# tzt101/MichiGAN

Hardware: NVIDIA H100
Metric: 512x512 images/sec (generator forward) (higher is better)
Workload: dtype fp16/bf16 tensor-core operands (bf16 hi+lo split where needed), fp32 accumulate and storage

## Files before the change

### michigan_b200/csrc/mg_aux.cu

```cuda
#include <cuda_runtime.h>
#include <cstdint>
#include <cmath>
#include <cstdlib>
#include <cuda_fp16.h>
#include <cuda_bf16.h>
#include "mg_internal.h"

namespace mg {

__device__ __forceinline__ float rtf32(float x) {
    uint32_t r;
    asm("cvt.rna.tf32.f32 %0, %1;\n" : "=r"(r) : "f"(x));
    return __uint_as_float(r);
}
__device__ __forceinline__ float act_fn(float v, int act) {
    if (act == MG_ACT_RELU) return fmaxf(v, 0.f);
    if (act == MG_ACT_LRELU) return v > 0.f ? v : 0.2f * v;
    if (act == MG_ACT_TANH) return tanhf(v);
    return v;
}
__device__ __forceinline__ void split16(float v, int fmt, uint16_t& hi, uint16_t& lo) {
    if (fmt == 1) {
        const __half h = __float2half_rn(fminf(fmaxf(v, -65504.f), 65504.f));
        hi = __half_as_ushort(h);
        lo = __half_as_ushort(__float2half_rn(v - __half2float(h)));
    } else {
        const __nv_bfloat16 h = __float2bfloat16_rn(v);
        hi = __bfloat16_as_ushort(h);
        lo = __bfloat16_as_ushort(__float2bfloat16_rn(v - __bfloat162float(h)));
    }
}
static inline int cdiv(long long a, long long b) { return (int)((a + b - 1) / b); }

__global__ void pack_weight_kernel(const float* __restrict__ w, float* __restrict__ out, int O, int I, int KH, int KW,
                                   const float* __restrict__ inv_sigma, int round_) {
    const long long total = (long long)O * KH * KW * I;
    const float s = inv_sigma ? *inv_sigma : 1.f;
    for (long long idx = blockIdx.x * (long long)blockDim.x + threadIdx.x; idx < total;
         idx += (long long)gridDim.x * blockDim.x) {
        const int i = idx % I;
        long long t = idx / I;
        const int kw = t % KW; t /= KW;
        const int kh = t % KH;
        const int o = t / KH;
        float v = w[(((long long)o * I + i) * KH + kh) * KW + kw] * s;
        out[idx] = round_ ? rtf32(v) : v;
    }
}

__global__ void pack_weight_gb_kernel(const float* __restrict__ wg, const float* __restrict__ wb,
                                      float* __restrict__ out, int C, int I, int KH, int KW, int BN) {
    const long long total = 2LL * C * KH * KW * I;
    const int half = BN / 2;
    for (long long idx = blockIdx.x * (long long)blockDim.x + threadIdx.x; idx < total;
         idx += (long long)gridDim.x * blockDim.x) {
        const int i = idx % I;
        long long t = idx / I;
        const int kw = t % KW; t /= KW;
        const int kh = t % KH;
        const int R = t / KH;
        const int tile = R / BN, rr = R % BN;
        const float* src = rr < half ? wg : wb;
        const int c = tile * half + (rr < half ? rr : rr - half);
        out[idx] = rtf32(src[(((long long)c * I + i) * KH + kh) * KW + kw]);
    }
}

__global__ void pack_weight16_kernel(const float* __restrict__ w, uint16_t* __restrict__ out, int O, int I, int KH, int KW,
                                     const float* __restrict__ inv_sigma, int fmt, int split) {
    const long long total = (long long)O * KH * KW * I;
    const float s = inv_sigma ? *inv_sigma : 1.f;
    const int parts = split ? 2 : 1;
    for (long long idx = blockIdx.x * (long long)blockDim.x + threadIdx.x; idx < total;
         idx += (long long)gridDim.x * blockDim.x) {
        const int i = idx % I;
        long long t = idx / I;
        const int kw = t % KW; t /= KW;
        const int kh = t % KH;
        const int o = t / KH;
        const float v = w[(((long long)o * I + i) * KH + kh) * KW + kw] * s;
        uint16_t hi, lo;
        split16(v, fmt, hi, lo);
        const size_t base = ((size_t)o * KH * KW + (size_t)(kh * KW + kw)) * parts * I;
        out[base + i] = hi;
        if (split) out[base + I + i] = lo;
    }
}
__global__ void pack_weight_gb16_kernel(const float* __restrict__ wg, const float* __restrict__ wb, uint16_t* __restrict__ out,
                                        int C, int I, int KH, int KW, int BN, int fmt, int split) {
    const long long total = 2LL * C * KH * KW * I;
    const int half = BN / 2;
    for (long long idx = blockIdx.x * (long long)blockDim.x + threadIdx.x; idx < total;
         idx += (long long)gridDim.x * blockDim.x) {
        const int i = idx % I;
        long long t = idx / I;
        const int kw = t % KW; t /= KW;
        const int kh = t % KH;
        const int R = t / KH;
        const int tile = R / BN, rr = R % BN;
        const float* src = rr < half ? wg : wb;
        const int c = tile * half + (rr < half ? rr : rr - half);
        uint16_t hi, lo;
        split16(src[(((long long)c * I + i) * KH + kh) * KW + kw], fmt, hi, lo);
        if (!split) {
            out[idx] = hi;
        } else {
            const size_t base = ((size_t)R * KH * KW + (size_t)(kh * KW + kw)) * 2 * I;
            out[base + i] = hi;
            out[base + I + i] = lo;
        }
    }
}

__global__ void pack_weight_thin_kernel(const float* __restrict__ w, float* __restrict__ out, int O, int I, int CinP,
                                        int KH, int KW) {
    const int total = KH * KW * CinP * O;
    for (int idx = blockIdx.x * blockDim.x + threadIdx.x; idx < total; idx += gridDim.x * blockDim.x) {
        const int o = idx % O;
        int t = idx / O;
        const int ci = t % CinP;
        const int tap = t / CinP;
        const int kh = tap / KW, kw = tap % KW;
        out[idx] = ci < I ? w[(((long long)o * I + ci) * KH + kh) * KW + kw] : 0.f;
    }
}

template <int CINP, int CPL>
__global__ void __launch_bounds__(256)
thin_conv_kernel(const mg_thin_args a, int tiles_w, int tiles_h, int num_tiles) {
    extern __shared__ __align__(16) float sm[];
    const int KH = a.KH, KW = a.KW, s = a.stride;
    const int Cout = a.Cout;
    const int PH = 7 * s + KH, PW = 15 * s + KW;
    float* w_s = sm;
    float* in_s = sm + KH * KW * CINP * Cout;
    const int nw = KH * KW * CINP * Cout;
    for (int i = threadIdx.x * 4; i < nw; i += blockDim.x * 4)
        *reinterpret_cast<float4*>(w_s + i) = __ldg(reinterpret_cast<const float4*>(a.w + i));

    const int warp = threadIdx.x >> 5, lane = threadIdx.x & 31;
    const int R = a.seg_resize > 0 ? a.seg_resize : 1;
    const int IH = a.H, IW = a.W;
    const int c_base = lane * CPL;
    const bool lane_active = c_base < Cout;

    for (int tile = blockIdx.x; tile < num_tiles; tile += gridDim.x) {
        const int tw = tile % tiles_w;
        const int th = (tile / tiles_w) % tiles_h;
        const int n = tile / (tiles_w * tiles_h);
        const int oh0 = th * 8, ow0 = tw * 16;
        const int ih0 = oh0 * s - a.pad, iw0 = ow0 * s - a.pad;
        __syncthreads();
        for (int i = threadIdx.x; i < PH * PW; i += blockDim.x) {
            const int py = i / PW, px = i - py * PW;
            int ih = ih0 + py, iw = iw0 + px;
            bool ok = true;
            if (a.pad_mode == 1) {
                if (ih < 0) ih = -ih;
                if (ih >= IH) ih = 2 * IH - 2 - ih;
                if (iw < 0) iw = -iw;
                if (iw >= IW) iw = 2 * IW - 2 - iw;
                ok = ih >= 0 && ih < IH && iw >= 0 && iw < IW;
            } else {
                ok = ih >= 0 && ih < IH && iw >= 0 && iw < IW;
            }
            float4 v0 = make_float4(0.f, 0.f, 0.f, 0.f), v1 = v0;
            if (ok) {
                const float* src = a.in + (((size_t)n * IH * R + (size_t)ih * R) * ((size_t)IW * R) + (size_t)iw * R) * CINP;
                v0 = __ldg(reinterpret_cast<const float4*>(src));
                if (CINP == 8) v1 = __ldg(reinterpret_cast<const float4*>(src + 4));
            }
            *reinterpret_cast<float4*>(in_s + (size_t)i * CINP) = v0;
            if (CINP == 8) *reinterpret_cast<float4*>(in_s + (size_t)i * CINP + 4) = v1;
        }
        __syncthreads();

        const int oh = oh0 + warp;
#pragma unroll 1
        for (int g = 0; g < 2; ++g) {
            float acc[8][CPL];
#pragma unroll
            for (int p_ = 0; p_ < 8; ++p_)
#pragma unroll
                for (int c = 0; c < CPL; ++c) acc[p_][c] = 0.f;
            if (lane_active) {
                for (int kh = 0; kh < KH; ++kh) {
                    const float* row = in_s + (size_t)((warp * s + kh) * PW) * CINP;
                    for (int kw = 0; kw < KW; ++kw) {
                        const float* wt = w_s + (size_t)((kh * KW + kw) * CINP) * Cout + c_base;
                        float wv[CINP][CPL];
#pragma unroll
                        for (int ci = 0; ci < CINP; ++ci) {
                            if constexpr (CPL == 4) {
                                const float4 t = *reinterpret_cast<const float4*>(wt + (size_t)ci * Cout);
                                wv[ci][0] = t.x; wv[ci][1] = t.y; wv[ci][2] = t.z; wv[ci][3] = t.w;
                            } else {
                                const float2 t = *reinterpret_cast<const float2*>(wt + (size_t)ci * Cout);
                                wv[ci][0] = t.x; wv[ci][1] = t.y;
                            }
                        }
#pragma unroll
                        for (int p_ = 0; p_ < 8; ++p_) {
                            const float* ip = row + (size_t)(((g * 8 + p_) * s + kw)) * CINP;
                            float iv[CINP];
                            const float4 t0 = *reinterpret_cast<const float4*>(ip);
                            iv[0] = t0.x; iv[1] = t0.y; iv[2] = t0.z; iv[3] = t0.w;
                            if constexpr (CINP == 8) {
                                const float4 t1 = *reinterpret_cast<const float4*>(ip + 4);
                                iv[4] = t1.x; iv[5] = t1.y; iv[6] = t1.z; iv[7] = t1.w;
                            }
#pragma unroll
                            for (int ci = 0; ci < CINP; ++ci)
#pragma unroll
                                for (int c = 0; c < CPL; ++c) acc[p_][c] = fmaf(iv[ci], wv[ci][c], acc[p_][c]);
                        }
                    }
                }
            }
            if (lane_active && oh < a.OH) {
                float bv[CPL];
#pragma unroll
                for (int c = 0; c < CPL; ++c) bv[c] = a.bias ? __ldg(a.bias + c_base + c) : 0.f;
#pragma unroll
                for (int p_ = 0; p_ < 8; ++p_) {
                    const int ow = ow0 + g * 8 + p_;
                    if (ow >= a.OW) continue;
                    const size_t pix = ((size_t)n * a.OH + oh) * a.OW + ow;
                    const float ps = a.pscale ? __ldg(a.pscale + pix) : 1.f;
                    const float pm = a.pmul ? __ldg(a.pmul + pix) : 1.f;
                    float y[CPL];
#pragma unroll
                    for (int c = 0; c < CPL; ++c) {
                        float v = act_fn(acc[p_][c] * ps + bv[c], a.act) * pm;
                        y[c] = a.round_out ? rtf32(v) : v;
                    }
                    if (a.out) {
                        float* op = a.out + pix * Cout + c_base;
                        if constexpr (CPL == 4) *reinterpret_cast<float4*>(op) = make_float4(y[0], y[1], y[2], y[3]);
                        else *reinterpret_cast<float2*>(op) = make_float2(y[0], y[1]);
                    }
                    if (a.out_hi) {
                        uint16_t hi[CPL], lo[CPL];
#pragma unroll
                        for (int c = 0; c < CPL; ++c) split16(y[c], a.out16_fmt, hi[c], lo[c]);
                        uint16_t* oh = reinterpret_cast<uint16_t*>(a.out_hi) + pix * Cout + c_base;
                        uint16_t* ol = a.out_lo ? reinterpret_cast<uint16_t*>(a.out_lo) + pix * Cout + c_base : nullptr;
                        if constexpr (CPL == 4) {
                            *reinterpret_cast<uint2*>(oh) = make_uint2(hi[0] | ((uint32_t)hi[1] << 16), hi[2] | ((uint32_t)hi[3] << 16));
                            if (ol) *reinterpret_cast<uint2*>(ol) = make_uint2(lo[0] | ((uint32_t)lo[1] << 16), lo[2] | ((uint32_t)lo[3] << 16));
                        } else {
                            *reinterpret_cast<uint32_t*>(oh) = hi[0] | ((uint32_t)hi[1] << 16);
                            if (ol) *reinterpret_cast<uint32_t*>(ol) = lo[0] | ((uint32_t)lo[1] << 16);
                        }
                    }
                }
            }
        }
    }
}


template <int CINP, int CPT>
__global__ void __launch_bounds__(256, 1)
thin_gemm_kernel(const mg_thin_args a, int tiles_w, int tiles_h, int num_tiles) {
    extern __shared__ __align__(16) float sm[];
    const int KH = a.KH, KW = a.KW, s = a.stride;
    constexpr int Cout = 16 * CPT;
    const int PH = 7 * s + KH, PW = 15 * s + KW;
    float* w_s = sm;
    float* in_s = sm + KH * KW * CINP * Cout;
    const int nw = KH * KW * CINP * Cout;
    for (int i = threadIdx.x * 4; i < nw; i += blockDim.x * 4)
        *reinterpret_cast<float4*>(w_s + i) = __ldg(reinterpret_cast<const float4*>(a.w + i));
    const int tx = threadIdx.x & 15, ty = threadIdx.x >> 4;
    const int prow = ty >> 1, pcol0 = (ty & 1) * 8;
    const int c_base = tx * CPT;
    const int R = a.seg_resize > 0 ? a.seg_resize : 1;
    const int IH = a.H, IW = a.W;
    float bv[CPT];
#pragma unroll
    for (int c = 0; c < CPT; ++c) bv[c] = a.bias ? __ldg(a.bias + c_base + c) : 0.f;

    for (int tile = blockIdx.x; tile < num_tiles; tile += gridDim.x) {
        const int tw = tile % tiles_w;
        const int th = (tile / tiles_w) % tiles_h;
        const int n = tile / (tiles_w * tiles_h);
        const int oh0 = th * 8, ow0 = tw * 16;
        const int ih0 = oh0 * s - a.pad, iw0 = ow0 * s - a.pad;
        __syncthreads();
        for (int i = threadIdx.x; i < PH * PW; i += blockDim.x) {
            const int py = i / PW, px = i - py * PW;
            int ih = ih0 + py, iw = iw0 + px;
            if (a.pad_mode == 1) {
                if (ih < 0) ih = -ih;
                if (ih >= IH) ih = 2 * IH - 2 - ih;
                if (iw < 0) iw = -iw;
                if (iw >= IW) iw = 2 * IW - 2 - iw;
            }
            const bool ok = ih >= 0 && ih < IH && iw >= 0 && iw < IW;
            float4 v0 = make_float4(0.f, 0.f, 0.f, 0.f), v1 = v0;
            if (ok) {
                const float* src = a.in + (((size_t)n * IH * R + (size_t)ih * R) * ((size_t)IW * R) + (size_t)iw * R) * CINP;
                v0 = __ldg(reinterpret_cast<const float4*>(src));
                if (CINP == 8) v1 = __ldg(reinterpret_cast<const float4*>(src + 4));
            }
            *reinterpret_cast<float4*>(in_s + (size_t)i * CINP) = v0;
            if (CINP == 8) *reinterpret_cast<float4*>(in_s + (size_t)i * CINP + 4) = v1;
        }
        __syncthreads();

        float acc[8][CPT];
#pragma unroll
        for (int p_ = 0; p_ < 8; ++p_)
#pragma unroll
            for (int c = 0; c < CPT; ++c) acc[p_][c] = 0.f;
        for (int kh = 0; kh < KH; ++kh) {
            const float* row = in_s + (size_t)((prow * s + kh) * PW) * CINP;
            for (int kw = 0; kw < KW; ++kw) {
                const float* wt = w_s + (size_t)((kh * KW + kw) * CINP) * Cout + c_base;
#pragma unroll
                for (int c4 = 0; c4 < CINP; c4 += 4) {
                    float wv[4][CPT];
#pragma unroll
                    for (int ci = 0; ci < 4; ++ci)
#pragma unroll
                        for (int c = 0; c < CPT; c += 4) {
                            const float4 t = *reinterpret_cast<const float4*>(wt + (size_t)(c4 + ci) * Cout + c);
                            wv[ci][c] = t.x; wv[ci][c + 1] = t.y; wv[ci][c + 2] = t.z; wv[ci][c + 3] = t.w;
                        }
#pragma unroll
                    for (int p_ = 0; p_ < 8; ++p_) {
                        const float4 iv = *reinterpret_cast<const float4*>(row + (size_t)((pcol0 + p_) * s + kw) * CINP + c4);
#pragma unroll
                        for (int c = 0; c < CPT; ++c) {
                            acc[p_][c] = fmaf(iv.x, wv[0][c], acc[p_][c]);
                            acc[p_][c] = fmaf(iv.y, wv[1][c], acc[p_][c]);
                            acc[p_][c] = fmaf(iv.z, wv[2][c], acc[p_][c]);
                            acc[p_][c] = fmaf(iv.w, wv[3][c], acc[p_][c]);
                        }
                    }
                }
            }
        }
        const int oh = oh0 + prow;
        if (oh < a.OH) {
#pragma unroll
            for (int p_ = 0; p_ < 8; ++p_) {
                const int ow = ow0 + pcol0 + p_;
                if (ow >= a.OW) continue;
                const size_t pix = ((size_t)n * a.OH + oh) * a.OW + ow;
                const float ps = a.pscale ? __ldg(a.pscale + pix) : 1.f;
                const float pm = a.pmul ? __ldg(a.pmul + pix) : 1.f;
                float y[CPT];
#pragma unroll
                for (int c = 0; c < CPT; ++c) {
                    const float v = act_fn(acc[p_][c] * ps + bv[c], a.act) * pm;
                    y[c] = a.round_out ? rtf32(v) : v;
                }
                if (a.out) {
                    float* op = a.out + pix * Cout + c_base;
#pragma unroll
                    for (int c = 0; c < CPT; c += 4) *reinterpret_cast<float4*>(op + c) = make_float4(y[c], y[c + 1], y[c + 2], y[c + 3]);
                }
                if (a.out_hi) {
                    uint16_t hi[CPT], lo[CPT];
#pragma unroll
                    for (int c = 0; c < CPT; ++c) split16(y[c], a.out16_fmt, hi[c], lo[c]);
                    uint16_t* ohp = reinterpret_cast<uint16_t*>(a.out_hi) + pix * Cout + c_base;
                    uint16_t* olp = a.out_lo ? reinterpret_cast<uint16_t*>(a.out_lo) + pix * Cout + c_base : nullptr;
#pragma unroll
                    for (int c = 0; c < CPT; c += 4) {
                        *reinterpret_cast<uint2*>(ohp + c) = make_uint2(hi[c] | ((uint32_t)hi[c + 1] << 16), hi[c + 2] | ((uint32_t)hi[c + 3] << 16));
                        if (olp) *reinterpret_cast<uint2*>(olp + c) = make_uint2(lo[c] | ((uint32_t)lo[c + 1] << 16), lo[c + 2] | ((uint32_t)lo[c + 3] << 16));
                    }
                }
            }
        }
    }
}

__global__ void __launch_bounds__(256)
conv_img_kernel(const float* __restrict__ x, const float* __restrict__ w, const float* __restrict__ bias,
                float* __restrict__ out, int N, int H, int W, int Cin, int Cout, int act_in, int act_out) {
    extern __shared__ __align__(16) float sm[];
    const int PW = 34, PH = 10, NP = PW * PH;
    const int C4 = Cin / 4;
    float* in_s = sm;
    float* w_s = sm + (size_t)C4 * NP * 4;
    for (int i = threadIdx.x; i < 9 * Cin * 4; i += blockDim.x) {
        const int co = i & 3;
        const int ci = (i >> 2) % Cin;
        const int tap = (i >> 2) / Cin;
        w_s[i] = co < Cout ? w[((size_t)co * Cin + ci) * 9 + tap] : 0.f;
    }
    const int tiles_w = (W + 31) / 32, tiles_h = (H + 7) / 8;
    const int tile = blockIdx.x;
    const int tw = tile % tiles_w, th = (tile / tiles_w) % tiles_h, n = tile / (tiles_w * tiles_h);
    const int h0 = th * 8 - 1, w0 = tw * 32 - 1;
    for (int i0 = threadIdx.x; i0 < NP * C4; i0 += 4 * blockDim.x) {
        float4 v[4];
#pragma unroll
        for (int u = 0; u < 4; ++u) {
            const int i = i0 + u * blockDim.x;
            const int c4 = i % C4, pp = i / C4;
            const int py = pp / PW, px = pp - py * PW;
            const int ih = h0 + py, iw = w0 + px;
            v[u] = make_float4(0.f, 0.f, 0.f, 0.f);
            if (i < NP * C4 && ih >= 0 && ih < H && iw >= 0 && iw < W)
                v[u] = __ldg(reinterpret_cast<const float4*>(x + (((size_t)n * H + ih) * W + iw) * Cin) + c4);
        }
#pragma unroll
        for (int u = 0; u < 4; ++u) {
            const int i = i0 + u * blockDim.x;
            if (i >= NP * C4) break;
            const int c4 = i % C4, pp = i / C4;
            const float4 r = make_float4(act_fn(v[u].x, act_in), act_fn(v[u].y, act_in), act_fn(v[u].z, act_in), act_fn(v[u].w, act_in));
            *reinterpret_cast<float4*>(in_s + ((size_t)c4 * NP + pp) * 4) = r;
        }
    }
    __syncthreads();
    const int ly = threadIdx.x >> 5, lx = threadIdx.x & 31;
    float a0 = 0.f, a1 = 0.f, a2 = 0.f;
    for (int kh = 0; kh < 3; ++kh)
        for (int kw = 0; kw < 3; ++kw) {
            const int pp = (ly + kh) * PW + lx + kw;
            const float* wt = w_s + (size_t)((kh * 3 + kw) * Cin) * 4;
#pragma unroll 4
            for (int c4 = 0; c4 < C4; ++c4) {
                const float4 v = *reinterpret_cast<const float4*>(in_s + ((size_t)c4 * NP + pp) * 4);
                const float4 w0v = *reinterpret_cast<const float4*>(wt + (c4 * 4 + 0) * 4);
                const float4 w1v = *reinterpret_cast<const float4*>(wt + (c4 * 4 + 1) * 4);
                const float4 w2v = *reinterpret_cast<const float4*>(wt + (c4 * 4 + 2) * 4);
                const float4 w3v = *reinterpret_cast<const float4*>(wt + (c4 * 4 + 3) * 4);
                a0 = fmaf(v.x, w0v.x, a0); a1 = fmaf(v.x, w0v.y, a1); a2 = fmaf(v.x, w0v.z, a2);
                a0 = fmaf(v.y, w1v.x, a0); a1 = fmaf(v.y, w1v.y, a1); a2 = fmaf(v.y, w1v.z, a2);
                a0 = fmaf(v.z, w2v.x, a0); a1 = fmaf(v.z, w2v.y, a1); a2 = fmaf(v.z, w2v.z, a2);
                a0 = fmaf(v.w, w3v.x, a0); a1 = fmaf(v.w, w3v.y, a1); a2 = fmaf(v.w, w3v.z, a2);
            }
        }
    const int oh = th * 8 + ly, ow = tw * 32 + lx;
    if (oh < H && ow < W) {
        const float r[3] = {a0, a1, a2};
        for (int co = 0; co < Cout; ++co)
            out[(((size_t)n * Cout + co) * H + oh) * W + ow] = act_fn(r[co] + (bias ? bias[co] : 0.f), act_out);
    }
}

__global__ void __launch_bounds__(256)
conv_to1_kernel(const float* __restrict__ x, const float* __restrict__ w, const float* __restrict__ bias,
                float* __restrict__ out, int N, int H, int W, int Cin, int KH, int KW, int pad, int OH, int OW) {
    extern __shared__ __align__(16) float w_s[];
    for (int i = threadIdx.x; i < KH * KW * Cin; i += blockDim.x) {
        const int ci = i % Cin, tap = i / Cin;
        w_s[i] = w[(size_t)ci * KH * KW + tap];
    }
    __syncthreads();
    const int warp = threadIdx.x >> 5, lane = threadIdx.x & 31;
    const long long total = (long long)N * OH * OW;
    for (long long o = blockIdx.x * 8LL + warp; o < total; o += gridDim.x * 8LL) {
        const int ow = o % OW;
        const int oh = (o / OW) % OH;
        const int n = o / ((long long)OW * OH);
        float acc = 0.f;
        for (int kh = 0; kh < KH; ++kh) {
            const int ih = oh + kh - pad;
            if (ih < 0 || ih >= H) continue;
            for (int kw = 0; kw < KW; ++kw) {
                const int iw = ow + kw - pad;
                if (iw < 0 || iw >= W) continue;
                const float4* xp = reinterpret_cast<const float4*>(x + (((size_t)n * H + ih) * W + iw) * Cin);
                const float4* wp = reinterpret_cast<const float4*>(w_s + (size_t)(kh * KW + kw) * Cin);
                for (int c4 = lane; c4 < Cin / 4; c4 += 32) {
                    const float4 a = __ldg(xp + c4);
                    const float4 b = wp[c4];
                    acc = fmaf(a.x, b.x, acc); acc = fmaf(a.y, b.y, acc);
                    acc = fmaf(a.z, b.z, acc); acc = fmaf(a.w, b.w, acc);
                }
            }
        }
#pragma unroll
        for (int off = 16; off > 0; off >>= 1) acc += __shfl_xor_sync(0xffffffffu, acc, off);
        if (lane == 0) out[o] = acc + (bias ? bias[0] : 0.f);
    }
}

__global__ void __launch_bounds__(256, 3)
chan_stats_kernel(const float* __restrict__ x, long long P, int C, double* __restrict__ sums, int blocks_per_b,
                  uint16_t* __restrict__ out16) {
    const int G = C / 4;
    const int tpr = G < 256 ? G : 256;
    const int rows = 256 / tpr;
    const int b = blockIdx.x / blocks_per_b;
    const int blk = blockIdx.x % blocks_per_b;
    const int tr = threadIdx.x / tpr, tc = threadIdx.x % tpr;
    const float* xb = x + (size_t)b * P * C;
    double* sb = sums + (size_t)b * 2 * C;
    __shared__ double red[256 * 8];
    for (int g0 = tc; g0 < G; g0 += tpr) {
        double s[4] = {0, 0, 0, 0}, q[4] = {0, 0, 0, 0};
        float fs[4] = {0, 0, 0, 0}, fq[4] = {0, 0, 0, 0};
        int cnt = 0;
        if (threadIdx.x < rows * tpr) {
            auto add = [&](const float4 v, long long pidx) {
                if (out16) {
                    const __nv_bfloat162 a = __floats2bfloat162_rn(v.x, v.y), bb = __floats2bfloat162_rn(v.z, v.w);
                    *reinterpret_cast<uint2*>(out16 + (size_t)pidx * C + g0 * 4) =
                        make_uint2(*reinterpret_cast<const uint32_t*>(&a), *reinterpret_cast<const uint32_t*>(&bb));
                }
                fs[0] += v.x; fs[1] += v.y; fs[2] += v.z; fs[3] += v.w;
                fq[0] = fmaf(v.x, v.x, fq[0]); fq[1] = fmaf(v.y, v.y, fq[1]);
                fq[2] = fmaf(v.z, v.z, fq[2]); fq[3] = fmaf(v.w, v.w, fq[3]);
                if (++cnt == 32) {
#pragma unroll
                    for (int i = 0; i < 4; ++i) { s[i] += fs[i]; q[i] += fq[i]; fs[i] = 0.f; fq[i] = 0.f; }
                    cnt = 0;
                }
            };
            const long long step = (long long)blocks_per_b * rows;
            long long pidx = (long long)blk * rows + tr;
            for (; pidx + 3 * step < P; pidx += 4 * step) {
                float4 v[4];
#pragma unroll
                for (int u = 0; u < 4; ++u) v[u] = __ldg(reinterpret_cast<const float4*>(xb + (size_t)(pidx + u * step) * C) + g0);
#pragma unroll
                for (int u = 0; u < 4; ++u) add(v[u], pidx + u * step);
            }
            for (; pidx < P; pidx += step) add(__ldg(reinterpret_cast<const float4*>(xb + (size_t)pidx * C) + g0), pidx);
#pragma unroll
            for (int i = 0; i < 4; ++i) { s[i] += fs[i]; q[i] += fq[i]; }
        }
        if (rows > 1) {
            __syncthreads();
#pragma unroll
            for (int i = 0; i < 4; ++i) { red[threadIdx.x * 8 + i] = s[i]; red[threadIdx.x * 8 + 4 + i] = q[i]; }
            __syncthreads();
            if (tr == 0) {
                for (int r = 1; r < rows; ++r)
#pragma unroll
                    for (int i = 0; i < 4; ++i) {
                        s[i] += red[(r * tpr + tc) * 8 + i];
                        q[i] += red[(r * tpr + tc) * 8 + 4 + i];
                    }
            }
        }
        if (tr == 0 && threadIdx.x < rows * tpr) {
#pragma unroll
            for (int i = 0; i < 4; ++i) {
                atomicAdd(sb + g0 * 4 + i, s[i]);
                atomicAdd(sb + C + g0 * 4 + i, q[i]);
            }
        }
    }
}

__global__ void bn_finalize_kernel(const double* __restrict__ sums, int C, double count, double unb_mult, float eps,
                                   float momentum, int clamp_mode, float* nscale, float* nshift, float* rmean,
                                   float* rvar, float* mean_out, float* var_out) {
    const int c = blockIdx.x * blockDim.x + threadIdx.x;
    if (c >= C) return;
    if (count <= 0.0) count = sums[2 * C];
    const double count_u = count * unb_mult;
    const double mean = sums[c] / count;
    double var = sums[C + c] / count - mean * mean;
    if (var < 0) var = 0;
    double rstd;
// ... 690 lines not shown
```

### michigan_b200/csrc/mg_wgrad.cu

```cuda
#include <cuda.h>
#include <cuda_runtime.h>
#include <cstdio>
#include <cstring>
#include <cstdlib>
#include "mg_ptx.cuh"
#include "mg_internal.h"

namespace mg {

constexpr int kWgThreads = 288;
constexpr int kWgStagesMax = 6;
constexpr int kWgMaxCols = 256;

struct WgradParams {
    int N, OH, OW, Cout, Cin, KH, KW, stride, pad;
    int TW, TH, TN, tiles_w, tiles_h, tiles_n, pix_tiles;
    int BN, m_tiles, n_tiles, splits, stages;
    int pix_tile, box_bytes;
    int f16;
    int kelem, mboxes, kmma;
    float* dw;
    double* dw64;
};

__device__ __forceinline__ uint32_t sw128(uint32_t k, uint32_t b) {
    const uint32_t o = k * 128 + b;
    return o ^ ((k & 7) << 4);
}

__device__ __forceinline__ void mma_tf32_16x8x8(float (&c)[4], const uint32_t (&a)[4], uint32_t b0, uint32_t b1) {
    asm volatile("mma.sync.aligned.m16n8k8.row.col.f32.tf32.tf32.f32 {%0, %1, %2, %3}, {%4, %5, %6, %7}, {%8, %9}, {%0, %1, %2, %3};\n"
                 : "+f"(c[0]), "+f"(c[1]), "+f"(c[2]), "+f"(c[3])
                 : "r"(a[0]), "r"(a[1]), "r"(a[2]), "r"(a[3]), "r"(b0), "r"(b1));
}
__device__ __forceinline__ void mma_bf16_16x8x16(float (&c)[4], const uint32_t (&a)[4], uint32_t b0, uint32_t b1) {
    asm volatile("mma.sync.aligned.m16n8k16.row.col.f32.bf16.bf16.f32 {%0, %1, %2, %3}, {%4, %5, %6, %7}, {%8, %9}, {%0, %1, %2, %3};\n"
                 : "+f"(c[0]), "+f"(c[1]), "+f"(c[2]), "+f"(c[3])
                 : "r"(a[0]), "r"(a[1]), "r"(a[2]), "r"(a[3]), "r"(b0), "r"(b1));
}

template <int KWT, int BNT>
__global__ void __launch_bounds__(kWgThreads, 1)
wgrad_tf32_kernel(const __grid_constant__ CUtensorMap tmDY, const __grid_constant__ CUtensorMap tmX, const WgradParams p) {
    extern __shared__ __align__(1024) uint8_t smem_raw[];
    uint8_t* smem = reinterpret_cast<uint8_t*>((reinterpret_cast<uintptr_t>(smem_raw) + 1023) & ~uintptr_t(1023));
    const int kBoxBytes = p.box_bytes;
    const int a_bytes = p.mboxes * kBoxBytes;
    const int b1_bytes = (p.BN / p.kelem) * kBoxBytes;
    const int stage_bytes = a_bytes + p.KW * b1_bytes;
    uint64_t* bars = reinterpret_cast<uint64_t*>(smem + (size_t)p.stages * stage_bytes);
    uint64_t* full_bar = bars;
    uint64_t* empty_bar = bars + kWgStagesMax;

    const int warp = threadIdx.x >> 5, lane = threadIdx.x & 31;
    const int n_units = p.KH * p.m_tiles * p.n_tiles;
    int u = blockIdx.x % n_units;
    const int split = blockIdx.x / n_units;
    const int nt = u % p.n_tiles; u /= p.n_tiles;
    const int mt = u % p.m_tiles;
    const int kh = u / p.m_tiles;
    const int t_begin = (int)((long long)p.pix_tiles * split / p.splits);
    const int t_end = (int)((long long)p.pix_tiles * (split + 1) / p.splits);

    if (warp == 8 && lane == 0) {
        tma_prefetch_desc(&tmDY);
        tma_prefetch_desc(&tmX);
        for (int s = 0; s < p.stages; ++s) { mbar_init(&full_bar[s], 1); mbar_init(&empty_bar[s], 8); }
        fence_barrier_init();
    }
    __syncthreads();

    if (warp == 8) {
        int st = 0; uint32_t ph = 0;
        const int nb_x = p.BN / p.kelem;
        const uint32_t tx = (uint32_t)stage_bytes;
        const int n_boxes = p.mboxes + p.KW * nb_x;
        for (int t = t_begin; t < t_end; ++t) {
            const int tw = t % p.tiles_w;
            const int th = (t / p.tiles_w) % p.tiles_h;
            const int tn = t / (p.tiles_w * p.tiles_h);
            const int ow0 = tw * p.TW, oh0 = th * p.TH, n0 = tn * p.TN;
            if (lane == 0) {
                mbar_wait_report(&empty_bar[st], ph ^ 1);
                mbar_arrive_expect_tx(&full_bar[st], tx);
            }
            __syncwarp();
            uint8_t* sa = smem + (size_t)st * stage_bytes;
            for (int b = lane; b < n_boxes; b += 32) {
                if (b < p.mboxes) {
                    tma_load_4d(sa + b * kBoxBytes, &tmDY, &full_bar[st], mt * 128 + b * p.kelem, ow0, oh0, n0);
                } else {
                    const int kw = (b - p.mboxes) / nb_x, j = (b - p.mboxes) - kw * nb_x;
                    tma_load_4d(sa + a_bytes + kw * b1_bytes + j * kBoxBytes, &tmX, &full_bar[st], nt * p.BN + j * p.kelem,
                                ow0 * p.stride - p.pad + kw, oh0 * p.stride - p.pad + kh, n0);
                }
            }
            __syncwarp();
            if (++st == p.stages) { st = 0; ph ^= 1; }
        }
    } else if constexpr (KWT > 0) {
        const int wg = warp >> 2;
        float acc[KWT][BNT / 2];
#pragma unroll
        for (int kw = 0; kw < KWT; ++kw)
#pragma unroll
            for (int i = 0; i < BNT / 2; ++i) acc[kw][i] = 0.f;
        int st = 0; uint32_t ph = 0;
        for (int t = t_begin; t < t_end; ++t) {
            mbar_wait(&full_bar[st], ph);
            const uint32_t sa = smem_u32(smem + (size_t)st * stage_bytes);
            const uint32_t a_base = sa + (uint32_t)(wg * kBoxBytes), b_base = sa + (uint32_t)a_bytes;
            wgmma_fence();
#pragma unroll 1
            for (int kk = 0; kk < p.pix_tile; kk += 16) {
                const uint64_t da = wg_desc_mn_sw128(a_base + (uint32_t)(kk * 128), (uint32_t)kBoxBytes);
#pragma unroll
                for (int kw = 0; kw < KWT; ++kw) {
                    const uint64_t db = wg_desc_mn_sw128(b_base + (uint32_t)(kw * b1_bytes + kk * 128), (uint32_t)kBoxBytes);
                    if constexpr (BNT == 128) wgmma_bf16_tt_n128(acc[kw], da, db, 1u);
                    else wgmma_bf16_tt_n64(acc[kw], da, db, 1u);
                }
            }
            wgmma_commit();
            wgmma_wait_all();
            __syncwarp();
            if (lane == 0) mbar_arrive(&empty_bar[st]);
            if (++st == p.stages) { st = 0; ph ^= 1; }
        }
        if (t_end > t_begin) {
            const int r0 = mt * 128 + wg * 64 + (warp & 3) * 16 + (lane >> 2), c0 = (lane & 3) * 2;
#pragma unroll
            for (int h = 0; h < 2; ++h) {
                const int co = r0 + 8 * h;
                if (co >= p.Cout) continue;
#pragma unroll
                for (int kw = 0; kw < KWT; ++kw)
#pragma unroll
                    for (int j = 0; j < BNT / 8; ++j) {
                        const size_t off = (size_t)co * (p.KH * KWT * p.Cin) + (size_t)(kh * KWT + kw) * p.Cin + nt * BNT + j * 8 + c0;
                        const float v0 = acc[kw][4 * j + 2 * h], v1 = acc[kw][4 * j + 2 * h + 1];
                        if (p.splits > 1) {
                            atomicAdd(p.dw64 + off, (double)v0);
                            atomicAdd(p.dw64 + off + 1, (double)v1);
                        } else {
                            *reinterpret_cast<float2*>(p.dw + off) = make_float2(v0, v1);
                        }
                    }
            }
        }
    } else {
        const int g = lane >> 2, t4 = lane & 3;
        const int m0 = warp * 16;
        const int ncols = p.KW * p.BN, n8 = ncols >> 3;
        const int esz = p.f16 ? 2 : 4;
        uint32_t a_off[2];
#pragma unroll
        for (int h = 0; h < 2; ++h) {
            const int m = m0 + g + 8 * h;
            a_off[h] = (uint32_t)((m / p.kelem) * kBoxBytes) | ((uint32_t)((m % p.kelem) * esz) << 20);
        }
        float acc[kWgMaxCols / 8][4];
#pragma unroll
        for (int j = 0; j < kWgMaxCols / 8; ++j) acc[j][0] = acc[j][1] = acc[j][2] = acc[j][3] = 0.f;
        int st = 0; uint32_t ph = 0;
        for (int t = t_begin; t < t_end; ++t) {
            mbar_wait(&full_bar[st], ph);
            const uint8_t* sa = smem + (size_t)st * stage_bytes;
            auto ldA = [&](int h, int k) -> const uint8_t* { return sa + (a_off[h] & 0xFFFFF) + sw128(k, a_off[h] >> 20); };
            for (int kk = 0; kk < p.pix_tile; kk += p.kmma) {
                uint32_t a[4];
                if (p.f16) {
#pragma unroll
                    for (int i = 0; i < 4; ++i) {
                        const int h = i & 1, k = kk + 2 * t4 + 8 * (i >> 1);
                        a[i] = (uint32_t)*reinterpret_cast<const uint16_t*>(ldA(h, k)) |
                               ((uint32_t)*reinterpret_cast<const uint16_t*>(ldA(h, k + 1)) << 16);
                    }
                } else {
#pragma unroll
                    for (int i = 0; i < 4; ++i) a[i] = *reinterpret_cast<const uint32_t*>(ldA(i & 1, kk + t4 + 4 * (i >> 1)));
                }
#pragma unroll
                for (int j = 0; j < kWgMaxCols / 8; ++j) {
                    if (j < n8) {
                        const int n = j * 8 + g, kw = n / p.BN, ci = n - kw * p.BN;
                        const uint8_t* bb = sa + a_bytes + kw * b1_bytes + (ci / p.kelem) * kBoxBytes;
                        const uint32_t cb = (uint32_t)((ci % p.kelem) * esz);
                        if (p.f16) {
                            const int k = kk + 2 * t4;
                            const uint32_t b0 = (uint32_t)*reinterpret_cast<const uint16_t*>(bb + sw128(k, cb)) |
                                                ((uint32_t)*reinterpret_cast<const uint16_t*>(bb + sw128(k + 1, cb)) << 16);
                            const uint32_t b1 = (uint32_t)*reinterpret_cast<const uint16_t*>(bb + sw128(k + 8, cb)) |
                                                ((uint32_t)*reinterpret_cast<const uint16_t*>(bb + sw128(k + 9, cb)) << 16);
                            mma_bf16_16x8x16(acc[j], a, b0, b1);
                        } else {
                            const uint32_t b0 = *reinterpret_cast<const uint32_t*>(bb + sw128(kk + t4, cb));
                            const uint32_t b1 = *reinterpret_cast<const uint32_t*>(bb + sw128(kk + t4 + 4, cb));
                            mma_tf32_16x8x8(acc[j], a, b0, b1);
                        }
                    }
                }
            }
            __syncwarp();
            if (lane == 0) mbar_arrive(&empty_bar[st]);
            if (++st == p.stages) { st = 0; ph ^= 1; }
        }
        if (t_end > t_begin) {
#pragma unroll
            for (int h = 0; h < 2; ++h) {
                const int co = mt * 128 + m0 + g + 8 * h;
                if (co >= p.Cout) continue;
#pragma unroll
                for (int j = 0; j < kWgMaxCols / 8; ++j) {
                    if (j < n8) {
                        const int n = j * 8 + 2 * t4, kw = n / p.BN, ci = n - kw * p.BN;
                        const size_t off = (size_t)co * (p.KH * p.KW * p.Cin) + (size_t)(kh * p.KW + kw) * p.Cin + nt * p.BN + ci;
                        if (p.splits > 1) {
                            atomicAdd(p.dw64 + off, (double)acc[j][2 * h]);
                            atomicAdd(p.dw64 + off + 1, (double)acc[j][2 * h + 1]);
                        } else {
                            *reinterpret_cast<float2*>(p.dw + off) = make_float2(acc[j][2 * h], acc[j][2 * h + 1]);
                        }
                    }
                }
            }
        }
    }
}

static int np2(int v) { int r = 1; while (r < v) r <<= 1; return r; }

}

using namespace mg;

static int wgrad_launch(const void* dy, const void* x, float* dw, int N, int H, int W, int Cin, int OH, int OW, int Cout,
                        int KH, int KW, int stride, int pad, int fmt, cudaStream_t stream) {
    if (!dy || !x || !dw) return set_error(-1, "mg_conv_wgrad: null pointer");
    if (fmt != 0 && fmt != 2) return set_error(-5, "mg_conv_wgrad: operand format must be 0 (tf32) or 2 (bf16)");
    const int kelem = fmt ? 64 : 32;
    if (Cin % kelem != 0 || Cout % kelem != 0) return set_error(-2, "mg_conv_wgrad: channels must be multiples of %d", kelem);
    WgradParams p;
    memset(&p, 0, sizeof(p));
    p.N = N; p.OH = OH; p.OW = OW; p.Cout = Cout; p.Cin = Cin; p.KH = KH; p.KW = KW; p.stride = stride; p.pad = pad;
    p.f16 = fmt; p.kelem = kelem; p.mboxes = 128 / kelem; p.kmma = fmt ? 16 : 8;
    int BN = Cin >= 128 ? 128 : Cin;
    if (Cin % BN != 0) BN = kelem;
    while (KW * BN > kWgMaxCols) BN /= 2;
    if (BN < kelem || Cin % BN != 0) return set_error(-3, "mg_conv_wgrad: KW %d x Cin %d does not fit the accumulator", KW, Cin);
    p.BN = BN;
    int pix_tile = 64;
    if ((200 * 1024) / ((p.mboxes + KW * (BN / kelem)) * 64 * 128) < 3) pix_tile = 32;
    p.pix_tile = pix_tile; p.box_bytes = pix_tile * 128;
    p.TW = np2(OW) < 8 ? np2(OW) : 8;
    int th = pix_tile / p.TW;
    p.TH = np2(OH) < th ? np2(OH) : th;
    p.TN = pix_tile / (p.TW * p.TH);
    p.tiles_w = (OW + p.TW - 1) / p.TW; p.tiles_h = (OH + p.TH - 1) / p.TH; p.tiles_n = (N + p.TN - 1) / p.TN;
    p.pix_tiles = p.tiles_w * p.tiles_h * p.tiles_n;
    p.m_tiles = (Cout + 127) / 128;
    p.n_tiles = Cin / BN;
    const int units = KH * p.m_tiles * p.n_tiles;
    int splits = (2 * num_sms()) / units;
    if (splits < 1) splits = 1;
    if (splits > p.pix_tiles) splits = p.pix_tiles;
    p.splits = splits;
    const int stage_bytes = p.mboxes * p.box_bytes + KW * (BN / kelem) * p.box_bytes;
    int stages = (200 * 1024) / stage_bytes;
    if (stages < 1) return set_error(-4, "mg_conv_wgrad: stage of %d bytes does not fit shared memory", stage_bytes);
    if (stages > kWgStagesMax) stages = kWgStagesMax;
    p.stages = stages;
    p.dw = dw;

    CUtensorMap tmDY, tmX;
    const int esz = fmt ? 2 : 4;
    const CUtensorMapDataType dt = fmt ? CU_TENSOR_MAP_DATA_TYPE_BFLOAT16 : CU_TENSOR_MAP_DATA_TYPE_FLOAT32;
    const CUtensorMapSwizzle sw = CU_TENSOR_MAP_SWIZZLE_128B;
    {
        cuuint64_t dims[4] = {(cuuint64_t)Cout, (cuuint64_t)OW, (cuuint64_t)OH, (cuuint64_t)N};
        cuuint64_t strides[3] = {(cuuint64_t)Cout * esz, (cuuint64_t)OW * Cout * esz, (cuuint64_t)OH * OW * Cout * esz};
        cuuint32_t box[4] = {(cuuint32_t)kelem, (cuuint32_t)p.TW, (cuuint32_t)p.TH, (cuuint32_t)p.TN};
        cuuint32_t es[4] = {1, 1, 1, 1};
        int rc = encode_tensor_map(&tmDY, (void*)dy, dt, 4, dims, strides, box, es, sw);
        if (rc) return rc;
    }
    {
        cuuint64_t dims[4] = {(cuuint64_t)Cin, (cuuint64_t)W, (cuuint64_t)H, (cuuint64_t)N};
        cuuint64_t strides[3] = {(cuuint64_t)Cin * esz, (cuuint64_t)W * Cin * esz, (cuuint64_t)H * W * Cin * esz};
        cuuint32_t box[4] = {(cuuint32_t)kelem, (cuuint32_t)(p.TW * stride), (cuuint32_t)(p.TH * stride), (cuuint32_t)p.TN};
        cuuint32_t es[4] = {1, (cuuint32_t)stride, (cuuint32_t)stride, 1};
        int rc = encode_tensor_map(&tmX, (void*)x, dt, 4, dims, strides, box, es, sw);
        if (rc) return rc;
    }
    void (*kern)(CUtensorMap, CUtensorMap, WgradParams) = wgrad_tf32_kernel<0, 0>;
    if (fmt == 2) {
        if (KW == 1 && BN == 64) kern = wgrad_tf32_kernel<1, 64>;
        else if (KW == 1 && BN == 128) kern = wgrad_tf32_kernel<1, 128>;
        else if (KW == 2 && BN == 64) kern = wgrad_tf32_kernel<2, 64>;
        else if (KW == 2 && BN == 128) kern = wgrad_tf32_kernel<2, 128>;
        else if (KW == 3 && BN == 64) kern = wgrad_tf32_kernel<3, 64>;
        else if (KW == 4 && BN == 64) kern = wgrad_tf32_kernel<4, 64>;
    }
    cudaError_t e = cudaFuncSetAttribute((const void*)kern, cudaFuncAttributeMaxDynamicSharedMemorySize, 227 * 1024);
    if (e != cudaSuccess) return set_error((int)e, "wgrad attr: %s", cudaGetErrorString(e));
    const size_t smem_bytes = (size_t)stages * stage_bytes + 1024 + 256;
    const size_t n_dw = (size_t)Cout * KH * KW * Cin;
    if (splits > 1) {
        const int rc = acc64_alloc(&p.dw64, n_dw, stream);
        if (rc) return rc;
    }
    kern<<<units * splits, kWgThreads, smem_bytes, stream>>>(tmDY, tmX, p);
    int rc = check_launch("mg_conv_wgrad");
    if (splits > 1) {
        if (!rc) rc = acc64_fold(p.dw64, dw, n_dw, 0, stream);
        const int rc2 = acc64_free(p.dw64, stream);
        if (!rc) rc = rc2;
    }
    return rc;
}

extern "C" int mg_conv_wgrad(const float* dy, const float* x, float* dw, int N, int H, int W, int Cin, int OH, int OW, int Cout,
                             int KH, int KW, int stride, int pad, void* stream_) {
    return wgrad_launch(dy, x, dw, N, H, W, Cin, OH, OW, Cout, KH, KW, stride, pad, 0, reinterpret_cast<cudaStream_t>(stream_));
}

extern "C" int mg_conv_wgrad16(const void* dy16, const void* x16, float* dw, int N, int H, int W, int Cin, int OH, int OW, int Cout,
                               int KH, int KW, int stride, int pad, void* stream_) {
    return wgrad_launch(dy16, x16, dw, N, H, W, Cin, OH, OW, Cout, KH, KW, stride, pad, 2, reinterpret_cast<cudaStream_t>(stream_));
}
```

Baseline: 212.1.

## Skip zero padded input channel in thin conv, widen image loads, specialize wgrad

The thin conv kernel now checks whether the padded last input channel's weights are all zero and, if so, runs a compile-time variant that skips those weight loads and FMAs. The image conv loader issues 11 outstanding float4 loads per iteration instead of 4 to raise memory-level parallelism. The TF32 wgrad path is templated on KW/BN with precomputed swizzle offsets and compile-time tile sizes, and the bf16 path in that general branch is dropped, so unsupported combinations now return an error. Only the first two changes affect the generator forward; the wgrad work is backward-only, and the extra load registers may cost occupancy.

```diff
diff --git a/michigan_b200/csrc/mg_aux.cu b/michigan_b200/csrc/mg_aux.cu
--- a/michigan_b200/csrc/mg_aux.cu
+++ b/michigan_b200/csrc/mg_aux.cu
@@ -1,4 +1,5 @@
 #include <cuda_runtime.h>
+#include <type_traits>
 #include <cstdint>
 #include <cmath>
 #include <cstdlib>
@@ -280,6 +281,11 @@
     float bv[CPT];
 #pragma unroll
     for (int c = 0; c < CPT; ++c) bv[c] = a.bias ? __ldg(a.bias + c_base + c) : 0.f;
+    __syncthreads();
+    bool zero_last = true;
+    for (int i = threadIdx.x; i < KH * KW * Cout; i += blockDim.x)
+        zero_last &= w_s[((i / Cout) * CINP + CINP - 1) * Cout + i % Cout] == 0.f;
+    const bool skip_last = __syncthreads_and(zero_last) != 0;
 
     for (int tile = blockIdx.x; tile < num_tiles; tile += gridDim.x) {
         const int tw = tile % tiles_w;
@@ -314,34 +320,42 @@
         for (int p_ = 0; p_ < 8; ++p_)
 #pragma unroll
             for (int c = 0; c < CPT; ++c) acc[p_][c] = 0.f;
-        for (int kh = 0; kh < KH; ++kh) {
-            const float* row = in_s + (size_t)((prow * s + kh) * PW) * CINP;
-            for (int kw = 0; kw < KW; ++kw) {
-                const float* wt = w_s + (size_t)((kh * KW + kw) * CINP) * Cout + c_base;
-#pragma unroll
-                for (int c4 = 0; c4 < CINP; c4 += 4) {
-                    float wv[4][CPT];
-#pragma unroll
-                    for (int ci = 0; ci < 4; ++ci)
-#pragma unroll
-                        for (int c = 0; c < CPT; c += 4) {
-                            const float4 t = *reinterpret_cast<const float4*>(wt + (size_t)(c4 + ci) * Cout + c);
-                            wv[ci][c] = t.x; wv[ci][c + 1] = t.y; wv[ci][c + 2] = t.z; wv[ci][c + 3] = t.w;
-                        }
-#pragma unroll
-                    for (int p_ = 0; p_ < 8; ++p_) {
-                        const float4 iv = *reinterpret_cast<const float4*>(row + (size_t)((pcol0 + p_) * s + kw) * CINP + c4);
-#pragma unroll
-                        for (int c = 0; c < CPT; ++c) {
-                            acc[p_][c] = fmaf(iv.x, wv[0][c], acc[p_][c]);
-                            acc[p_][c] = fmaf(iv.y, wv[1][c], acc[p_][c]);
-                            acc[p_][c] = fmaf(iv.z, wv[2][c], acc[p_][c]);
-                            acc[p_][c] = fmaf(iv.w, wv[3][c], acc[p_][c]);
+        auto mac = [&](auto skip) {
+            constexpr bool SKIP = decltype(skip)::value;
+            for (int kh = 0; kh < KH; ++kh) {
+                const float* row = in_s + (size_t)((prow * s + kh) * PW) * CINP;
+                for (int kw = 0; kw < KW; ++kw) {
+                    const float* wt = w_s + (size_t)((kh * KW + kw) * CINP) * Cout + c_base;
+#pragma unroll
+                    for (int c4 = 0; c4 < CINP; c4 += 4) {
+                        constexpr int kLast = CINP - 4;
+                        const bool part = SKIP && c4 == kLast;
+                        float wv[4][CPT];
+#pragma unroll
+                        for (int ci = 0; ci < 4; ++ci)
+#pragma unroll
+                            for (int c = 0; c < CPT; c += 4) {
+                                if (part && ci == 3) continue;
+                                const float4 t = *reinterpret_cast<const float4*>(wt + (size_t)(c4 + ci) * Cout + c);
+                                wv[ci][c] = t.x; wv[ci][c + 1] = t.y; wv[ci][c + 2] = t.z; wv[ci][c + 3] = t.w;
+                            }
+#pragma unroll
+                        for (int p_ = 0; p_ < 8; ++p_) {
+                            const float4 iv = *reinterpret_cast<const float4*>(row + (size_t)((pcol0 + p_) * s + kw) * CINP + c4);
+#pragma unroll
+                            for (int c = 0; c < CPT; ++c) {
+                                acc[p_][c] = fmaf(iv.x, wv[0][c], acc[p_][c]);
+                                acc[p_][c] = fmaf(iv.y, wv[1][c], acc[p_][c]);
+                                acc[p_][c] = fmaf(iv.z, wv[2][c], acc[p_][c]);
+                                if (!part) acc[p_][c] = fmaf(iv.w, wv[3][c], acc[p_][c]);
+                            }
                         }
                     }
                 }
             }
-        }
+        };
+        if (skip_last) mac(std::true_type{});
+        else mac(std::false_type{});
         const int oh = oh0 + prow;
         if (oh < a.OH) {
 #pragma unroll
@@ -397,10 +411,11 @@
     const int tile = blockIdx.x;
     const int tw = tile % tiles_w, th = (tile / tiles_w) % tiles_h, n = tile / (tiles_w * tiles_h);
     const int h0 = th * 8 - 1, w0 = tw * 32 - 1;
-    for (int i0 = threadIdx.x; i0 < NP * C4; i0 += 4 * blockDim.x) {
-        float4 v[4];
-#pragma unroll
-        for (int u = 0; u < 4; ++u) {
+    constexpr int kLoads = 11;
+    for (int i0 = threadIdx.x; i0 < NP * C4; i0 += kLoads * blockDim.x) {
+        float4 v[kLoads];
+#pragma unroll
+        for (int u = 0; u < kLoads; ++u) {
             const int i = i0 + u * blockDim.x;
             const int c4 = i % C4, pp = i / C4;
             const int py = pp / PW, px = pp - py * PW;
@@ -410,7 +425,7 @@
                 v[u] = __ldg(reinterpret_cast<const float4*>(x + (((size_t)n * H + ih) * W + iw) * Cin) + c4);
         }
 #pragma unroll
-        for (int u = 0; u < 4; ++u) {
+        for (int u = 0; u < kLoads; ++u) {
             const int i = i0 + u * blockDim.x;
             if (i >= NP * C4) break;
             const int c4 = i % C4, pp = i / C4;
diff --git a/michigan_b200/csrc/mg_wgrad.cu b/michigan_b200/csrc/mg_wgrad.cu
--- a/michigan_b200/csrc/mg_wgrad.cu
+++ b/michigan_b200/csrc/mg_wgrad.cu
@@ -23,23 +23,14 @@
     double* dw64;
 };
 
-__device__ __forceinline__ uint32_t sw128(uint32_t k, uint32_t b) {
-    const uint32_t o = k * 128 + b;
-    return o ^ ((k & 7) << 4);
-}
+__host__ __device__ constexpr int wg_pix_tile(int boxes) { return (200 * 1024) / (boxes * 64 * 128) < 3 ? 32 : 64; }
 
 __device__ __forceinline__ void mma_tf32_16x8x8(float (&c)[4], const uint32_t (&a)[4], uint32_t b0, uint32_t b1) {
     asm volatile("mma.sync.aligned.m16n8k8.row.col.f32.tf32.tf32.f32 {%0, %1, %2, %3}, {%4, %5, %6, %7}, {%8, %9}, {%0, %1, %2, %3};\n"
                  : "+f"(c[0]), "+f"(c[1]), "+f"(c[2]), "+f"(c[3])
                  : "r"(a[0]), "r"(a[1]), "r"(a[2]), "r"(a[3]), "r"(b0), "r"(b1));
 }
-__device__ __forceinline__ void mma_bf16_16x8x16(float (&c)[4], const uint32_t (&a)[4], uint32_t b0, uint32_t b1) {
-    asm volatile("mma.sync.aligned.m16n8k16.row.col.f32.bf16.bf16.f32 {%0, %1, %2, %3}, {%4, %5, %6, %7}, {%8, %9}, {%0, %1, %2, %3};\n"
-                 : "+f"(c[0]), "+f"(c[1]), "+f"(c[2]), "+f"(c[3])
-                 : "r"(a[0]), "r"(a[1]), "r"(a[2]), "r"(a[3]), "r"(b0), "r"(b1));
-}
-
-template <int KWT, int BNT>
+template <int FMT, int KWT, int BNT>
 __global__ void __launch_bounds__(kWgThreads, 1)
 wgrad_tf32_kernel(const __grid_constant__ CUtensorMap tmDY, const __grid_constant__ CUtensorMap tmX, const WgradParams p) {
     extern __shared__ __align__(1024) uint8_t smem_raw[];
@@ -98,7 +89,7 @@
             __syncwarp();
             if (++st == p.stages) { st = 0; ph ^= 1; }
         }
-    } else if constexpr (KWT > 0) {
+    } else if constexpr (FMT == 2) {
         const int wg = warp >> 2;
         float acc[KWT][BNT / 2];
 #pragma unroll
@@ -149,56 +140,47 @@
             }
         }
     } else {
+        constexpr int kNb = BNT / 32;
+        constexpr int kPix = wg_pix_tile(4 + KWT * kNb);
+        constexpr int kBox = kPix * 128, kA = 4 * kBox, kB1 = kNb * kBox, kStage = kA + KWT * kB1;
+        constexpr int kN8 = KWT * BNT / 8;
+        static_assert(BNT % 32 == 0 && kN8 <= kWgMaxCols / 8, "TF32 wgrad tile");
         const int g = lane >> 2, t4 = lane & 3;
         const int m0 = warp * 16;
-        const int ncols = p.KW * p.BN, n8 = ncols >> 3;
-        const int esz = p.f16 ? 2 : 4;
-        uint32_t a_off[2];
-#pragma unroll
-        for (int h = 0; h < 2; ++h) {
-            const int m = m0 + g + 8 * h;
-            a_off[h] = (uint32_t)((m / p.kelem) * kBoxBytes) | ((uint32_t)((m % p.kelem) * esz) << 20);
-        }
-        float acc[kWgMaxCols / 8][4];
-#pragma unroll
-        for (int j = 0; j < kWgMaxCols / 8; ++j) acc[j][0] = acc[j][1] = acc[j][2] = acc[j][3] = 0.f;
+        const uint8_t* ssm = smem_raw + ((0u - smem_u32(smem_raw)) & 1023u);
+        uint32_t a_off[4];
+#pragma unroll
+        for (int i = 0; i < 4; ++i) {
+            const uint32_t r = (uint32_t)(t4 + 4 * (i >> 1)), m = (uint32_t)(m0 + g + 8 * (i & 1));
+            a_off[i] = (m / 32) * kBox + r * 128 + (((m % 32) * 4) ^ (r << 4));
+        }
+        uint32_t b_off[4][2];
+#pragma unroll
+        for (int jj = 0; jj < 4; ++jj)
+#pragma unroll
+            for (int q = 0; q < 2; ++q) {
+                const uint32_t r = (uint32_t)(t4 + 4 * q);
+                b_off[jj][q] = r * 128 + ((uint32_t)(16 * jj + 4 * (g & 3) + 64 * (g >> 2)) ^ (r << 4));
+            }
+        float acc[kN8][4];
+#pragma unroll
+        for (int j = 0; j < kN8; ++j) acc[j][0] = acc[j][1] = acc[j][2] = acc[j][3] = 0.f;
         int st = 0; uint32_t ph = 0;
         for (int t = t_begin; t < t_end; ++t) {
             mbar_wait(&full_bar[st], ph);
-            const uint8_t* sa = smem + (size_t)st * stage_bytes;
-            auto ldA = [&](int h, int k) -> const uint8_t* { return sa + (a_off[h] & 0xFFFFF) + sw128(k, a_off[h] >> 20); };
-            for (int kk = 0; kk < p.pix_tile; kk += p.kmma) {
+            const uint8_t* sa = ssm + st * kStage;
+#pragma unroll
+            for (int kk = 0; kk < kPix; kk += 8) {
                 uint32_t a[4];
-                if (p.f16) {
-#pragma unroll
-                    for (int i = 0; i < 4; ++i) {
-                        const int h = i & 1, k = kk + 2 * t4 + 8 * (i >> 1);
-                        a[i] = (uint32_t)*reinterpret_cast<const uint16_t*>(ldA(h, k)) |
-                               ((uint32_t)*reinterpret_cast<const uint16_t*>(ldA(h, k + 1)) << 16);
-                    }
-                } else {
-#pragma unroll
-                    for (int i = 0; i < 4; ++i) a[i] = *reinterpret_cast<const uint32_t*>(ldA(i & 1, kk + t4 + 4 * (i >> 1)));
-                }
-#pragma unroll
-                for (int j = 0; j < kWgMaxCols / 8; ++j) {
-                    if (j < n8) {
-                        const int n = j * 8 + g, kw = n / p.BN, ci = n - kw * p.BN;
-                        const uint8_t* bb = sa + a_bytes + kw * b1_bytes + (ci / p.kelem) * kBoxBytes;
-                        const uint32_t cb = (uint32_t)((ci % p.kelem) * esz);
-                        if (p.f16) {
-                            const int k = kk + 2 * t4;
-                            const uint32_t b0 = (uint32_t)*reinterpret_cast<const uint16_t*>(bb + sw128(k, cb)) |
-                                                ((uint32_t)*reinterpret_cast<const uint16_t*>(bb + sw128(k + 1, cb)) << 16);
-                            const uint32_t b1 = (uint32_t)*reinterpret_cast<const uint16_t*>(bb + sw128(k + 8, cb)) |
-                                                ((uint32_t)*reinterpret_cast<const uint16_t*>(bb + sw128(k + 9, cb)) << 16);
-                            mma_bf16_16x8x16(acc[j], a, b0, b1);
-                        } else {
-                            const uint32_t b0 = *reinterpret_cast<const uint32_t*>(bb + sw128(kk + t4, cb));
-                            const uint32_t b1 = *reinterpret_cast<const uint32_t*>(bb + sw128(kk + t4 + 4, cb));
-                            mma_tf32_16x8x8(acc[j], a, b0, b1);
-                        }
-                    }
+#pragma unroll
+                for (int i = 0; i < 4; ++i) a[i] = *reinterpret_cast<const uint32_t*>(sa + a_off[i] + kk * 128);
+#pragma unroll
+                for (int j = 0; j < kN8; ++j) {
+                    const int kw = j / (BNT / 8), jb = j % (BNT / 8);
+                    const uint8_t* bb = sa + kA + kw * kB1 + (jb / 4) * kBox + kk * 128;
+                    const uint32_t b0 = *reinterpret_cast<const uint32_t*>(bb + b_off[jb % 4][0]);
+                    const uint32_t b1 = *reinterpret_cast<const uint32_t*>(bb + b_off[jb % 4][1]);
+                    mma_tf32_16x8x8(acc[j], a, b0, b1);
                 }
             }
             __syncwarp();
@@ -206,21 +188,21 @@
             if (++st == p.stages) { st = 0; ph ^= 1; }
         }
         if (t_end > t_begin) {
+            const int cq = 2 * (t4 & 1) + 16 * (t4 >> 1);
 #pragma unroll
             for (int h = 0; h < 2; ++h) {
                 const int co = mt * 128 + m0 + g + 8 * h;
                 if (co >= p.Cout) continue;
 #pragma unroll
-                for (int j = 0; j < kWgMaxCols / 8; ++j) {
-                    if (j < n8) {
-                        const int n = j * 8 + 2 * t4, kw = n / p.BN, ci = n - kw * p.BN;
-                        const size_t off = (size_t)co * (p.KH * p.KW * p.Cin) + (size_t)(kh * p.KW + kw) * p.Cin + nt * p.BN + ci;
-                        if (p.splits > 1) {
-                            atomicAdd(p.dw64 + off, (double)acc[j][2 * h]);
-                            atomicAdd(p.dw64 + off + 1, (double)acc[j][2 * h + 1]);
-                        } else {
-                            *reinterpret_cast<float2*>(p.dw + off) = make_float2(acc[j][2 * h], acc[j][2 * h + 1]);
-                        }
+                for (int j = 0; j < kN8; ++j) {
+                    const int kw = j / (BNT / 8), jb = j % (BNT / 8);
+                    const int ci = (jb / 4) * 32 + 4 * (jb % 4) + cq;
+                    const size_t off = (size_t)co * (p.KH * KWT * p.Cin) + (size_t)(kh * KWT + kw) * p.Cin + nt * BNT + ci;
+                    if (p.splits > 1) {
+                        atomicAdd(p.dw64 + off, (double)acc[j][2 * h]);
+                        atomicAdd(p.dw64 + off + 1, (double)acc[j][2 * h + 1]);
+                    } else {
+                        *reinterpret_cast<float2*>(p.dw + off) = make_float2(acc[j][2 * h], acc[j][2 * h + 1]);
                     }
                 }
             }
@@ -249,8 +231,7 @@
     while (KW * BN > kWgMaxCols) BN /= 2;
     if (BN < kelem || Cin % BN != 0) return set_error(-3, "mg_conv_wgrad: KW %d x Cin %d does not fit the accumulator", KW, Cin);
     p.BN = BN;
-    int pix_tile = 64;
-    if ((200 * 1024) / ((p.mboxes + KW * (BN / kelem)) * 64 * 128) < 3) pix_tile = 32;
+    const int pix_tile = wg_pix_tile(p.mboxes + KW * (BN / kelem));
     p.pix_tile = pix_tile; p.box_bytes = pix_tile * 128;
     p.TW = np2(OW) < 8 ? np2(OW) : 8;
     int th = pix_tile / p.TW;
@@ -292,15 +273,24 @@
         int rc = encode_tensor_map(&tmX, (void*)x, dt, 4, dims, strides, box, es, sw);
         if (rc) return rc;
     }
-    void (*kern)(CUtensorMap, CUtensorMap, WgradParams) = wgrad_tf32_kernel<0, 0>;
+    void (*kern)(CUtensorMap, CUtensorMap, WgradParams) = nullptr;
     if (fmt == 2) {
-        if (KW == 1 && BN == 64) kern = wgrad_tf32_kernel<1, 64>;
-        else if (KW == 1 && BN == 128) kern = wgrad_tf32_kernel<1, 128>;
-        else if (KW == 2 && BN == 64) kern = wgrad_tf32_kernel<2, 64>;
-        else if (KW == 2 && BN == 128) kern = wgrad_tf32_kernel<2, 128>;
-        else if (KW == 3 && BN == 64) kern = wgrad_tf32_kernel<3, 64>;
-        else if (KW == 4 && BN == 64) kern = wgrad_tf32_kernel<4, 64>;
-    }
+        if (KW == 1 && BN == 64) kern = wgrad_tf32_kernel<2, 1, 64>;
+        else if (KW == 1 && BN == 128) kern = wgrad_tf32_kernel<2, 1, 128>;
+        else if (KW == 2 && BN == 64) kern = wgrad_tf32_kernel<2, 2, 64>;
+        else if (KW == 2 && BN == 128) kern = wgrad_tf32_kernel<2, 2, 128>;
+        else if (KW == 3 && BN == 64) kern = wgrad_tf32_kernel<2, 3, 64>;
+        else if (KW == 4 && BN == 64) kern = wgrad_tf32_kernel<2, 4, 64>;
+    } else {
+        if (KW == 1 && BN == 32) kern = wgrad_tf32_kernel<0, 1, 32>;
+        else if (KW == 1 && BN == 64) kern = wgrad_tf32_kernel<0, 1, 64>;
+        else if (KW == 1 && BN == 128) kern = wgrad_tf32_kernel<0, 1, 128>;
+        else if (KW == 3 && BN == 32) kern = wgrad_tf32_kernel<0, 3, 32>;
+        else if (KW == 3 && BN == 64) kern = wgrad_tf32_kernel<0, 3, 64>;
+        else if (KW == 4 && BN == 32) kern = wgrad_tf32_kernel<0, 4, 32>;
+        else if (KW == 4 && BN == 64) kern = wgrad_tf32_kernel<0, 4, 64>;
+    }
+    if (!kern) return set_error(-3, "mg_conv_wgrad: no %s kernel for KW %d x BN %d", fmt ? "bf16" : "TF32", KW, BN);
     cudaError_t e = cudaFuncSetAttribute((const void*)kern, cudaFuncAttributeMaxDynamicSharedMemorySize, 227 * 1024);
     if (e != cudaSuccess) return set_error((int)e, "wgrad attr: %s", cudaGetErrorString(e));
     const size_t smem_bytes = (size_t)stages * stage_bytes + 1024 + 256;
```

Measured after the change: 213.4, median of 6. No clear change (+0.6%).
